# hyx1999/SAM-Decoding

Measured on AMD Instinct MI355X. Metric: tokens/sec (+ mean accepted tokens), Vicuna-7B bs=1, samd_sam_only draft+verify, higher is better.
Workload: dtype f16

## Files before the change

include/samd_hip.h:

```cpp
#ifndef SAMD_HIP_H
#define SAMD_HIP_H

#include <stdint.h>

#ifdef __cplusplus
extern "C" {
#endif

#define SAMD_OK 0
#define SAMD_E_INVALID (-1)
#define SAMD_E_CAPACITY (-2)
#define SAMD_E_HIP (-3)
#define SAMD_E_IO (-4)
#define SAMD_E_NODEVICE (-5)

#define SAMD_MAX_DRAFT 128
#define SAMD_TOPK 8

#define SAMD_REP_DMETA 0
#define SAMD_REP_VERDICT 16
#define SAMD_REP_TOKENS 24
#define SAMD_REP_KVINDEX 152
#define SAMD_REP_COUNTERS 280
#define SAMD_REP_META 288
// ... 135 lines not shown

int samd_session_accept(samd_session_t *s, const int32_t *d_node_argmax, void *stream);
int samd_session_candidates(samd_session_t *s, int64_t *d_candidates, int32_t *d_rowmap, int32_t capacity, void *stream);
int samd_session_step_given(samd_session_t *s, const samd_static_t *sam, const samd_params_t *p, const int32_t *d_best_accept,
                            const int32_t *d_next_token, void *stream);
int samd_session_read_verdict(samd_session_t *s, samd_verdict_host_t *out, void *stream);
int samd_session_commit(samd_session_t *s, const samd_static_t *sam, void *stream);
int samd_session_step(samd_session_t *s, const samd_static_t *sam, const samd_params_t *p,
                      const int32_t *d_node_argmax, void *stream);

int samd_posterior_sampled(const void *d_probs, int32_t dtype, const int64_t *d_candidates, int32_t n_candidates, int32_t depth, int64_t vocab,
                           const double *d_uniforms, int32_t n_uniforms, void *d_work, int32_t *d_out, void *stream);
int samd_posterior_sampled_nodes(const void *d_probs, int32_t dtype, const int32_t *d_rowmap, int32_t n_rows, const int64_t *d_candidates,
                                 int32_t n_candidates, int32_t depth, int64_t vocab, const double *d_uniforms, int32_t n_uniforms,
                                 void *d_work, int32_t *d_out, void *stream);
int samd_kv_compact(samd_session_t *s, void *const *d_tensors, int32_t n_tensors, int32_t n_heads, int64_t max_len,
                    int32_t head_dim, int32_t elem_bytes, void *stream);

int samd_kv_compact_indices(void *const *d_tensors, int32_t n_tensors, int32_t n_heads, int64_t max_len, int32_t head_dim,
                            int32_t elem_bytes, int32_t start, const int32_t *d_indices, int32_t accept, void *stream);

int samd_session_set_cache_length(samd_session_t *s, int32_t length, void *stream);
int samd_session_get_cache_length(samd_session_t *s, int32_t *h_out, void *stream);

typedef struct samd_warm {
    const void *d_packed_w;
    int32_t N, K, splits;
    int32_t kb_per_workgroup;
    int32_t delay;
    int32_t where;
} samd_warm_t;

int64_t samd_tree_attention_workspace(int32_t n_q_pad, int32_t n_heads, int32_t head_dim);
int samd_tree_attention(const void *d_q, const void *d_k_cache, const void *d_v_cache, void *d_out, int32_t dtype,
                        int32_t n_q_pad, int32_t n_heads, int32_t n_kv_heads, int32_t head_dim, int64_t max_len,
                        const uint64_t *d_mask, const int32_t *d_cache_length, const int32_t *d_n, float scale,
                        void *d_workspace, int64_t workspace_bytes, void *stream);
int samd_tree_attention_vt(const void *d_q, const void *d_k_cache, const void *d_vt_cache, void *d_out, int32_t dtype,
                           int32_t n_q_pad, int32_t n_heads, int32_t n_kv_heads, int32_t head_dim, int64_t max_len,
                           const uint64_t *d_mask, const int32_t *d_cache_length, const int32_t *d_n, float scale,
                           void *d_workspace, int64_t workspace_bytes, const samd_warm_t *next, void *stream);
int samd_tree_attention_warm(const void *d_q, const void *d_k_cache, const void *d_v_cache, void *d_out, int32_t dtype,
                             int32_t n_q_pad, int32_t n_heads, int32_t n_kv_heads, int32_t head_dim, int64_t max_len,
                             const uint64_t *d_mask, const int32_t *d_cache_length, const int32_t *d_n, float scale,
                             void *d_workspace, int64_t workspace_bytes, const samd_warm_t *next, void *stream);

// ... 177 lines not shown
```

sam-decoding_amd/csrc/sam_device.h:

```cpp
#pragma once
#include <hip/hip_runtime.h>
#include "samd_common.h"

#define WAVE 64
#define PATH_PAD 255

__device__ __forceinline__ int lane_id() { return threadIdx.x & (WAVE - 1); }

__device__ __forceinline__ void wave_mem_sync() { __builtin_amdgcn_fence(__ATOMIC_SEQ_CST, "workgroup"); }

__device__ __forceinline__ int spill_search(const SamEdge *tab, int deg, int tok) {
    const uint32_t m = samd_spill_slots(deg);
    uint32_t h = samd_spill_hash(tok, m);
    for (uint32_t probes = 0; probes < m; probes++) {
        const SamEdge e = tab[h];
        if (e.tok == tok) return e.dst;
        if (e.tok == -1) return -1;
        h = (h + 1) & (m - 1);
    }
    return -1;
}

__device__ __forceinline__ int st_transfer(const StaticDev &S, int &idx, int &len, int tok) {
    int visited = 0;
// ... 752 lines not shown
            type = 0;
            if (md >= ms || !have_static) {
                int a = id;
                if (a != 0) {
                    const int maxlen = D.meta[M_MAXLEN];
                    int to_end = maxlen - D.minend[a];
                    while (D.link[a] != 0 && P.n_predicts > to_end) { a = D.link[a]; to_end = maxlen - D.minend[a]; }
                }
                n = seq_draft_fixed(sh, D.text, D.meta[M_NTEXT], D.minend[a], P.n_predicts, start);
            } else {
                n = seq_draft_fixed(sh, S.text, S.n_text, S.nodes[is].aux, P.n_predicts, start);
            }
        } else {
            type = 2; n = 1;
            if (lane_id() == 0) { sh.tokens[0] = start; sh.parent[0] = -1; }
            __syncthreads();
        }
    }
    int nl, mxd;
    build_buffers(sh, n, 0, nl, mxd);
    store_draft(D, sh, type, n, nl, mxd, id, md, is, ms, 0);
}

__device__ __forceinline__ void do_accept(const SessionDev &D, StepShared &sh, const int *node_argmax, int type, int n,
                                          int n_leaves, int max_depth, int &accept_out, int &next_token_out) {
    const int i = lane_id();
    for (int k = i; k < n; k += WAVE) sh.node_argmax[k] = node_argmax[k];
    __syncthreads();
    int key = -1;
    for (int row = i; row < n_leaves; row += WAVE) {
        int acc = 0;
        for (int j = 1; j < max_depth; j++) {
            const int cj = sh.path[row][j], pj = sh.path[row][j - 1];
            const int cand = cj == PATH_PAD ? 0 : sh.tokens[cj];
            const int am = sh.node_argmax[pj == PATH_PAD ? n - 1 : pj];
            if (cand != am) break;
            acc++;
        }
        const int kk = acc * SAMD_MAX_DRAFT + (SAMD_MAX_DRAFT - 1 - row);
        key = kk > key ? kk : key;
    }
    for (int o = 32; o > 0; o >>= 1) { int v = __shfl_xor(key, o); key = v > key ? v : key; }
    const int best_acc = key / SAMD_MAX_DRAFT, best = SAMD_MAX_DRAFT - 1 - (key % SAMD_MAX_DRAFT);
    const int a = best_acc + 1;
    for (int k = i; k < a; k += WAVE) {
        const int node = sh.path[best][k];
        const int tk = node == PATH_PAD ? 0 : sh.tokens[node];
        sh.accepted[k] = tk;
        D.acc_tokens[k] = tk;
        D.kv_index[k] = node == PATH_PAD ? -1 : node;
    }
    const int nn_raw = sh.path[best][best_acc];
    const int nn = nn_raw == PATH_PAD ? n - 1 : nn_raw;
    const int next_token = sh.node_argmax[nn];
    if (i == 0) {
        const int start = D.cache_length[0];
        D.verdict[V_BEST] = best; D.verdict[V_ACCEPT] = a; D.verdict[V_NEXT_NODE] = nn; D.verdict[V_NEXT_TOKEN] = next_token;
        D.verdict[V_KV_START] = start; D.verdict[V_IS_TREE] = (type != 0);
        D.cache_length[0] = start + a;
        D.start_token[0] = next_token;
        D.counters[C_STEPS] += 1; D.counters[C_TOKENS] += a;
        D.counters[type == 0 ? C_SEQ_STEPS : C_TREE_STEPS] += 1;
    }
    __syncthreads();
    accept_out = a; next_token_out = next_token;
}

__device__ __forceinline__ void do_accept_given(const SessionDev &D, StepShared &sh, const int *given, const int *next_token_ptr, int type, int n,
                                                int n_leaves, int max_depth, int &accept_out, int &next_token_out) {
    const int i = lane_id();
    int best = given[0], a = given[1];
    best = best < 0 ? 0 : (best >= n_leaves ? (n_leaves > 0 ? n_leaves - 1 : 0) : best);
    a = a < 1 ? 1 : (a > max_depth ? max_depth : a);
    for (int k = i; k < a; k += WAVE) {
        const int node = sh.path[best][k];
        const int tk = node == PATH_PAD ? 0 : sh.tokens[node];
        sh.accepted[k] = tk;
        D.acc_tokens[k] = tk;
        D.kv_index[k] = node == PATH_PAD ? -1 : node;
    }
    const int nn_raw = sh.path[best][a - 1];
    const int nn = nn_raw == PATH_PAD ? n - 1 : nn_raw;
    const int next_token = next_token_ptr[0];
    if (i == 0) {
        const int start = D.cache_length[0];
        D.verdict[V_BEST] = best; D.verdict[V_ACCEPT] = a; D.verdict[V_NEXT_NODE] = nn; D.verdict[V_NEXT_TOKEN] = next_token;
        D.verdict[V_KV_START] = start; D.verdict[V_IS_TREE] = (type != 0);
        D.cache_length[0] = start + a;
        D.start_token[0] = next_token;
        D.counters[C_STEPS] += 1; D.counters[C_TOKENS] += a;
        D.counters[type == 0 ? C_SEQ_STEPS : C_TREE_STEPS] += 1;
    }
    __syncthreads();
    accept_out = a; next_token_out = next_token;
}
```

sam-decoding_amd/csrc/sam_kernels.hip:

```cpp
#include <hip/hip_runtime.h>
#include <cstdio>
#include <cstdlib>
#include <cstring>
#include <ctime>
#include <functional>
#include <vector>
#include <hipcub/hipcub.hpp>
#include "sam_device.h"

#define HIPCHK(x) do { hipError_t e_ = (x); if (e_ != hipSuccess) { samd_set_error("%s: %s", #x, hipGetErrorString(e_)); return SAMD_E_HIP; } } while (0)
#define LAUNCHCHK() do { hipError_t e_ = hipGetLastError(); if (e_ != hipSuccess) { samd_set_error("kernel launch: %s", hipGetErrorString(e_)); return SAMD_E_HIP; } } while (0)

static inline StaticDev static_view(const samd_static_t *s) {
    StaticDev v;
    if (!s) { memset(&v, 0, sizeof(v)); return v; }
    v.nodes = s->d_nodes; v.root_next = s->d_root; v.spill = s->d_spill; v.text = s->d_text;
    v.n_states = (int32_t)s->n_states; v.vocab = (int32_t)s->vocab; v.n_text = (int32_t)s->n_text; v.kind = s->kind;
    v.chain = (const uint4 *)s->d_chain; v.chain_w = samd_chain_w(s->vocab);
    v.root16 = (const uint4 *)s->d_root16; v.bigram = (const uint4 *)s->d_d1hash; v.bigram_mask = s->n_d1hash > 0 ? (uint32_t)(s->n_d1hash - 1) : 0u;
    v.rc_bits = (const uint32_t *)s->d_rc_bits;
    v.ehash = (const uint4 *)s->d_ehash; v.edge_mask = s->n_ehash > 0 ? (uint32_t)(s->n_ehash - 1) : 0u;
    v.topk_cnt = (const int32_t *)s->d_topk_cnt;
    v.hot = s->d_d1hash ? (const uint4 *)s->d_hot : nullptr; v.blocks = s->d_d1hash ? (const uint4 *)s->d_blocks : nullptr; v.eb_tok_bits = samd_eb_tok_bits(s->vocab);
    return v;
// ... 75 lines not shown
    const int32_t *node_argmax;
    const int32_t *given;
    const int32_t *given_next;
    int index, match, start, source, type, reverse;
    int c0, c1, c2, c3;
    int have_static;
    int only_if_deferred;
    int push_report;
};

__device__ __forceinline__ void load_draft(const SessionDev &D, StepShared &sh, int &type, int &n, int &nl, int &md) {
    const int i = lane_id();
    type = D.dmeta[D_TYPE]; n = D.dmeta[D_N]; nl = D.dmeta[D_NLEAVES]; md = D.dmeta[D_MAXDEPTH];
    for (int k = i; k < n; k += WAVE) { sh.tokens[k] = D.tokens[k]; sh.parent[k] = D.parent[k]; }
    path_fill(sh, nl < SAMD_MAX_DRAFT ? (nl < 1 ? 1 : nl) : SAMD_MAX_DRAFT);
    __syncthreads();
    for (int k = i; k < nl * md; k += WAVE) {
        const int v = D.retrieve[k];
        sh.path[k / md][k % md] = v < 0 ? PATH_PAD : (unsigned char)v;
    }
    __syncthreads();
}

__global__ __launch_bounds__(64) void k_session(SessionDev D, StaticDev S, samd_params_t P, StepArgs A) {
    __shared__ StepShared sh;
    const int lane = lane_id();

    if (A.ops & OP_RESET) {
        for (uint32_t k = lane; k <= D.hmask; k += WAVE) D.hkey[k] = SAMD_HEMPTY;
        if (lane == 0) {
            D.link[0] = -1; D.length[0] = 0; D.minend[0] = 0; D.head[0] = -1; D.tail[0] = -1;
            D.text[0] = -1;
            for (int k = 0; k < M_COUNT; k++) D.meta[k] = 0;
            D.meta[M_NSTATES] = 1; D.meta[M_NTEXT] = 1;
            for (int k = 0; k < D_COUNT; k++) D.dmeta[k] = 0;
            for (int k = 0; k < V_COUNT; k++) D.verdict[k] = 0;
            for (int k = 0; k < C_COUNT; k++) D.counters[k] = 0;
            D.start_token[0] = 0; D.cache_length[0] = 0;
        }
        wave_mem_sync();
    }
    if (A.ops & OP_SET_CURSORS) {
        if (lane == 0) { D.meta[M_CUR_IDX] = A.c0; D.meta[M_CUR_LEN] = A.c1; D.meta[M_ST_IDX] = A.c2; D.meta[M_ST_LEN] = A.c3; }
        wave_mem_sync();
    }
    int n_in = A.d_n ? A.d_n[0] : A.n;
    unsigned long long t_prev = __builtin_amdgcn_s_memrealtime();
    auto phase_done = [&](int slot) {
// ... 65 lines not shown
    if (A.ops & OP_DRAFT_FIXED) {
        int n;
        if (A.source == 0) {
            int a = A.index;
            if (a != 0) {
                const int maxlen = D.meta[M_MAXLEN];
                int to_end = maxlen - D.minend[a];
                while (D.link[a] != 0 && P.n_predicts > to_end) { a = D.link[a]; to_end = maxlen - D.minend[a]; }
            }
            n = seq_draft_fixed(sh, D.text, D.meta[M_NTEXT], D.minend[a], P.n_predicts, A.start);
            if (lane == 0) D.dmeta[9] = a;
        } else {
            n = seq_draft_fixed(sh, S.text, S.n_text, S.nodes[A.index].aux, P.n_predicts, A.start);
        }
        int nl, mxd; build_buffers(sh, n, 0, nl, mxd);
        store_draft(D, sh, 0, n, nl, mxd, A.index, 0, A.index, 0, 0);
    }
    if ((A.ops & OP_SET_DRAFT) && !(A.only_if_deferred && D.dmeta[D_TYPE] != 2)) {
        for (int k = lane; k < A.n; k += WAVE) { sh.tokens[k] = A.tokens[k]; sh.parent[k] = A.parents[k]; }
        __syncthreads();
        int nl, mxd; build_buffers(sh, A.n, A.reverse, nl, mxd);
        store_draft(D, sh, A.type, A.n, nl, mxd, 0, 0, 0, 0, A.reverse);
    }
    if (A.push_report && D.h_report) {
        wave_mem_sync();
        for (int k = lane; k < SAMD_REPORT_INTS; k += WAVE)
            __hip_atomic_store(D.h_report + k, D.dmeta[k], __ATOMIC_RELAXED, __HIP_MEMORY_SCOPE_SYSTEM);
        __builtin_amdgcn_fence(__ATOMIC_RELEASE, "");
        asm volatile("s_waitcnt vmcnt(0)" ::: "memory");
        if (lane == 0) {
            const int seq = D.push_seq[0] + 1;
            D.push_seq[0] = seq;
            __hip_atomic_store(D.h_report + SAMD_REPORT_INTS, seq, __ATOMIC_RELEASE, __HIP_MEMORY_SCOPE_SYSTEM);
        }
    }
}

__global__ __launch_bounds__(64) void k_tree_buffers(const int32_t *parent, int n, int reverse, int32_t *position, uint64_t *mask,
                                                     uint8_t *mask_bool, int32_t *retrieve, int32_t *shape) {
    __shared__ StepShared sh;
    const int i = lane_id();
    for (int k = i; k < n; k += WAVE) sh.parent[k] = parent[k];
    __syncthreads();
    int nl, md; build_buffers(sh, n, reverse, nl, md);
    for (int k = i; k < n; k += WAVE) {
        if (position) position[k] = sh.position[k];
        if (mask) { mask[k] = sh.mask[k]; if (n > 64) mask[n + k] = sh.mask_hi[k]; }
        if (mask_bool) for (int j = 0; j < n; j++) mask_bool[(size_t)k * n + j] = (uint8_t)(((j < 64 ? sh.mask[k] >> j : sh.mask_hi[k] >> (j - 64))) & 1ull);
    }
    if (retrieve) for (int k = i; k < nl * md; k += WAVE) { const unsigned char v = sh.path[k / md][k % md]; retrieve[k] = v == PATH_PAD ? -1 : (int)v; }
    if (shape && i == 0) { shape[0] = nl; shape[1] = md; }
}

__global__ __launch_bounds__(64) void k_scripted_argmax(SessionDev D, const int32_t *__restrict__ target, int n_target, int vocab,
                                                        int32_t *__restrict__ out) {
    __shared__ int tok[SAMD_MAX_DRAFT], par[SAMD_MAX_DRAFT];
    const int i = lane_id();
    const int n = D.dmeta[D_N];
// ... 561 lines not shown
    if (!d_visited) return SAMD_E_INVALID;
    return walk_streams(sam, d_cursors, d_tokens, B, T, commit, nullptr, d_visited, stream);
}

int samd_session_create(int32_t max_tokens, samd_session_t **out) {
    if (!out || max_tokens < 1 || max_tokens > (1 << 24)) { samd_set_error("samd_session_create: invalid max_tokens"); return SAMD_E_INVALID; }
    if (samd_device_count() < 1) { samd_set_error("no HIP device"); return SAMD_E_NODEVICE; }
    samd_session_t *s = (samd_session_t *)calloc(1, sizeof(samd_session_t));
    if (!s) { samd_set_error("out of host memory"); return SAMD_E_CAPACITY; }
    s->max_tokens = max_tokens;
    SessionDev &D = s->dev;
    D.max_tokens = max_tokens;
    D.cap_states = 2 * max_tokens + 2;
    D.cap_text = max_tokens + 2;
    uint32_t H = 1024; while (H < (uint32_t)max_tokens * 8u) H <<= 1;
    D.hmask = H - 1;
    size_t off = 0;
    auto carve = [&](size_t bytes) { size_t o = off; off = align_up(off + bytes, 256); return o; };
    const size_t o_link = carve(4ull * D.cap_states), o_len = carve(4ull * D.cap_states), o_me = carve(4ull * D.cap_states),
                 o_head = carve(4ull * D.cap_states), o_tail = carve(4ull * D.cap_states), o_hk = carve(8ull * H),
                 o_hd = carve(4ull * H), o_hn = carve(4ull * H), o_text = carve(4ull * D.cap_text),
                 o_tok = carve(4 * SAMD_MAX_DRAFT), o_par = carve(4 * SAMD_MAX_DRAFT), o_pos = carve(4 * SAMD_MAX_DRAFT), o_mask = carve(8 * 2 * SAMD_MAX_DRAFT),
                 o_ret = carve(4 * SAMD_MAX_DRAFT * SAMD_MAX_DRAFT),
                 o_rep = carve(4 * SAMD_REPORT_INTS), o_st = carve(4), o_cl = carve(4), o_seq = carve(4);
    s->arena_bytes = off;
    if (hipMalloc(&s->arena, off) != hipSuccess) { free(s); samd_set_error("hipMalloc(session arena) failed"); return SAMD_E_HIP; }
    char *base = (char *)s->arena;
    D.link = (int32_t *)(base + o_link); D.length = (int32_t *)(base + o_len); D.minend = (int32_t *)(base + o_me);
    D.head = (int32_t *)(base + o_head); D.tail = (int32_t *)(base + o_tail); D.hkey = (uint64_t *)(base + o_hk);
    D.hdst = (int32_t *)(base + o_hd); D.hnext = (int32_t *)(base + o_hn); D.text = (int32_t *)(base + o_text);
    D.tokens = (int32_t *)(base + o_tok); D.parent = (int32_t *)(base + o_par);
    D.position = (int32_t *)(base + o_pos); D.mask = (uint64_t *)(base + o_mask); D.mask_hi = D.mask + SAMD_MAX_DRAFT; D.retrieve = (int32_t *)(base + o_ret);
    int32_t *rep = (int32_t *)(base + o_rep);
    D.dmeta = rep + SAMD_REP_DMETA; D.verdict = rep + SAMD_REP_VERDICT; D.acc_tokens = rep + SAMD_REP_TOKENS;
    D.kv_index = rep + SAMD_REP_KVINDEX; D.counters = rep + SAMD_REP_COUNTERS; D.meta = rep + SAMD_REP_META;
    D.start_token = (int32_t *)(base + o_st); D.cache_length = (int32_t *)(base + o_cl);
    D.push_seq = (int32_t *)(base + o_seq); D.h_report = nullptr;
    if (hipMemset(s->arena, 0, off) != hipSuccess) { (void)hipFree(s->arena); free(s); return SAMD_E_HIP; }
    *out = s;
    int32_t *target = nullptr;
    int rc = samd_session_report_target(s, &target);
    if (rc == SAMD_OK) rc = samd_session_reset(s, nullptr);
    if (rc == SAMD_OK && hipStreamSynchronize(nullptr) != hipSuccess) rc = SAMD_E_HIP;
    if (rc) { samd_session_free(s); *out = nullptr; }
    return rc;
}

void samd_session_free(samd_session_t *s) {
    if (!s) return;
    if (s->arena) (void)hipFree(s->arena);
    if (s->h_report_host) (void)hipHostFree(s->h_report_host);
    free(s);
}

int samd_session_report_target(samd_session_t *s, int32_t **out_host) {
    if (!s || !out_host) return SAMD_E_INVALID;
    if (!s->h_report_host) {
        void *h = nullptr, *d = nullptr;
        const size_t bytes = 4 * (SAMD_REPORT_INTS + 16);
        if (hipHostMalloc(&h, bytes, hipHostMallocCoherent | hipHostMallocMapped) != hipSuccess) { samd_set_error("hipHostMalloc(report target) failed"); return SAMD_E_HIP; }
// ... 9 lines not shown
int samd_report_wait(const int32_t *h_report, int32_t last_seq, int64_t timeout_us) {
    if (!h_report) return SAMD_E_INVALID;
    const volatile int32_t *seq = h_report + SAMD_REPORT_INTS;
    timespec t0; clock_gettime(CLOCK_MONOTONIC, &t0);
    for (unsigned spin = 0;; spin++) {
        if (*seq != last_seq) { __atomic_thread_fence(__ATOMIC_ACQUIRE); return SAMD_OK; }
        __builtin_ia32_pause();
        if ((spin & 1023u) == 1023u) {
            timespec t; clock_gettime(CLOCK_MONOTONIC, &t);
            if ((t.tv_sec - t0.tv_sec) * 1000000ll + (t.tv_nsec - t0.tv_nsec) / 1000 > timeout_us) return SAMD_E_CAPACITY;
        }
    }
}

static int launch_session(samd_session_t *s, const samd_static_t *sam, const samd_params_t *p, StepArgs &A, void *stream) {
    if (!s) { samd_set_error("null session"); return SAMD_E_INVALID; }
    if (sam && !sam->uploaded) { samd_set_error("static automaton not uploaded"); return SAMD_E_INVALID; }
    samd_params_t P; memset(&P, 0, sizeof(P));
    if (p) P = *p;
    if (p && (P.max_predicts > SAMD_MAX_DRAFT || P.n_predicts > SAMD_MAX_DRAFT || P.max_predicts < 0 || P.n_predicts < 0)) {
        samd_set_error("max_predicts / n_predicts must be in [0, %d]", SAMD_MAX_DRAFT); return SAMD_E_INVALID;
    }
    A.have_static = sam ? 1 : 0;
    hipLaunchKernelGGL(k_session, dim3(1), dim3(WAVE), 0, (hipStream_t)stream, s->dev, static_view(sam), P, A);
    LAUNCHCHK();
    return SAMD_OK;
}

int samd_session_reset(samd_session_t *s, void *stream) {
    StepArgs A; memset(&A, 0, sizeof(A)); A.ops = OP_RESET;
    return launch_session(s, nullptr, nullptr, A, stream);
}

int samd_dyn_add_tokens(samd_session_t *s, const int32_t *d_tokens, int32_t n, const int32_t *d_n, void *stream) {
    if (n < 0 || (!d_tokens && n > 0)) return SAMD_E_INVALID;
    StepArgs A; memset(&A, 0, sizeof(A)); A.ops = OP_ADD; A.tokens = d_tokens; A.n = n; A.d_n = d_n;
    return launch_session(s, nullptr, nullptr, A, stream);
}

int samd_dyn_walk(samd_session_t *s, const int32_t *d_tokens, int32_t n, int32_t commit, int32_t *d_out, void *stream) {
    if (n < 0 || (!d_tokens && n > 0)) return SAMD_E_INVALID;
    StepArgs A; memset(&A, 0, sizeof(A)); A.ops = OP_DYN_WALK; A.tokens = d_tokens; A.n = n; A.commit = commit; A.out2 = d_out;
    return launch_session(s, nullptr, nullptr, A, stream);
}

int samd_session_static_walk(samd_session_t *s, const samd_static_t *sam, const int32_t *d_tokens, int32_t n,
                             const int32_t *d_n, int32_t commit, int32_t *d_out, void *stream) {
// ... 147 lines not shown
        D2H(hk.data(), D.hkey, 8 * H); D2H(hd.data(), D.hdst, 4 * H); D2H(hn.data(), D.hnext, 4 * H); D2H(head.data(), D.head, 4ull * ns);
        HIPCHK(hipStreamSynchronize((hipStream_t)stream));
        size_t k = 0;
        for (int st = 0; st < ns; st++) {
            int d = 0;
            for (int e = head[st]; e >= 0; e = hn[e]) {
                if (h_edge_tok) h_edge_tok[k] = (int32_t)(uint32_t)hk[e];
                if (h_edge_dst) h_edge_dst[k] = hd[e];
                k++; d++;
            }
            if (h_deg) h_deg[st] = d;
        }
    }
    HIPCHK(hipStreamSynchronize((hipStream_t)stream));
    return SAMD_OK;
}

int samd_session_set_cache_length(samd_session_t *s, int32_t length, void *stream) {
    if (!s || length < 0) return SAMD_E_INVALID;
    HIPCHK(hipMemsetD32Async((hipDeviceptr_t)s->dev.cache_length, length, 1, (hipStream_t)stream));
    return SAMD_OK;
}

int samd_session_get_cache_length(samd_session_t *s, int32_t *h_out, void *stream) {
    if (!s || !h_out) return SAMD_E_INVALID;
    D2H(h_out, s->dev.cache_length, 4);
    HIPCHK(hipStreamSynchronize((hipStream_t)stream));
    return SAMD_OK;
}

int samd_scripted_argmax(samd_session_t *s, const int32_t *d_target, int32_t n_target, int32_t vocab, int32_t *d_out, void *stream) {
    if (!s || !d_target || !d_out || n_target < 0 || vocab < 4) return SAMD_E_INVALID;
    hipLaunchKernelGGL(k_scripted_argmax, dim3(1), dim3(WAVE), 0, (hipStream_t)stream, s->dev, d_target, n_target, vocab, d_out);
    LAUNCHCHK();
    return SAMD_OK;
}

static int scripted_logits(samd_session_t *s, const int32_t *d_argmax, void *d_logits, int32_t dtype, int32_t rows, int64_t row_stride, int32_t markov_vocab,
                           int order, void *stream) {
    if (!s || !d_argmax || !d_logits || markov_vocab < 4 || row_stride < markov_vocab) return SAMD_E_INVALID;
    hipStream_t st = (hipStream_t)stream;
#define SCRIPTED(T) do { if (order == 2) hipLaunchKernelGGL((k_scripted_logits<T, 2>), dim3(SAMD_MAX_DRAFT), dim3(WAVE), 0, st, s->dev, d_argmax, (T *)d_logits, (long long)row_stride, markov_vocab, rows); \
                         else hipLaunchKernelGGL((k_scripted_logits<T, 1>), dim3(SAMD_MAX_DRAFT), dim3(WAVE), 0, st, s->dev, d_argmax, (T *)d_logits, (long long)row_stride, markov_vocab, rows); } while (0)
    if (dtype == SAMD_F16) SCRIPTED(_Float16);
    else if (dtype == SAMD_BF16) SCRIPTED(__bf16);
    else if (dtype == SAMD_F32) SCRIPTED(float);
// ... 26 lines not shown
```

sam-decoding_amd/csrc/samd_common.h:

```cpp
#pragma once
#include <stdint.h>
#include <stddef.h>
#include "../../include/samd_hip.h"

#define SAMD_ABI_VERSION 2
#define SAMD_INLINE_EDGES 5
#define SAMD_SPILL_HEAD 3

#define SAMD_SINGLE 0x40000000
#define SAMD_RUN 0x20000000
#define SAMD_LEN_MASK 0x1FFFFFFF
struct __attribute__((aligned(64))) SamNode {
    int32_t link, length, e0_tok, e0_dst;
    int32_t aux, deg, e1_tok, e1_dst;
    int32_t e2_tok, e2_dst, e3_tok, e3_dst;
    int32_t e4_tok, e4_dst, spill, reserved;
};
static_assert(sizeof(SamNode) == 64, "SamNode must be one 64-byte line");
#define SAMD_EDGE_WORD(k) ((k) == 0 ? 2 : 4 + 2 * (k))

struct SamEdge { int32_t tok, dst; };

#if defined(__HIPCC__)
#define SAMD_HD __host__ __device__
// ... 60 lines not shown
enum { C_STEPS = 0, C_TOKENS, C_SEQ_STEPS, C_TREE_STEPS, C_T_ACCEPT, C_T_DYN, C_T_STATIC, C_T_DRAFT, C_COUNT = 8 };

#define SAMD_HEMPTY 0xFFFFFFFFFFFFFFFFull

struct SessionDev {
    int32_t *link, *length, *minend, *head, *tail;
    uint64_t *hkey;
    int32_t *hdst, *hnext;
    int32_t *text;
    int32_t *meta;
    int32_t *tokens, *parent, *position;
    uint64_t *mask;
    uint64_t *mask_hi;
    int32_t *retrieve;
    int32_t *dmeta;
    int32_t *verdict;
    int32_t *acc_tokens, *kv_index;
    int32_t *start_token, *cache_length;
    int32_t *counters;
    uint32_t hmask;
    int32_t cap_states, cap_text, max_tokens;
    int32_t *h_report;
    int32_t *push_seq;
};

struct samd_session {
    SessionDev dev;
    void *arena;
    size_t arena_bytes;
    int32_t max_tokens;
    int32_t *h_report_host;
};

struct samd_static {
    int32_t kind;
    int64_t n_states, n_edges, n_spill, vocab, n_text;
    SamNode *h_nodes;
    int32_t *h_root;
    SamEdge *h_spill;
    int32_t *h_text;
    SamNode *d_nodes;
    int32_t *d_root;
    SamEdge *d_spill;
    int32_t *d_text;
    int uploaded;
    int borrowed;
    void *d_chain;
// ... 58 lines not shown
```

sam-decoding_amd/samd_hip/__init__.py:

```python
import ctypes as C
import os

import numpy as np

_HERE = os.path.dirname(os.path.abspath(__file__))
LIB_PATH = os.environ.get("SAMD_HIP_LIB") or os.path.join(_HERE, "libsamd_hip.so")
MAX_DRAFT = 128
TILE_ROWS = 64
TOPK = 8
REP_DMETA, REP_VERDICT, REP_TOKENS, REP_KVINDEX, REP_COUNTERS, REP_META, REPORT_INTS = 0, 16, 24, 152, 280, 288, 304
KIND_COUNT, KIND_ENDPOS = 0, 1
F16, BF16, F32 = 0, 1, 2

_lib = None


class SamdError(RuntimeError):
    pass


class Params(C.Structure):
    _fields_ = [("variant", C.c_int32), ("max_predicts", C.c_int32), ("alpha", C.c_double), ("K", C.c_int32),
                ("len_bias", C.c_int32), ("n_predicts", C.c_int32), ("len_threshold", C.c_int32),
                ("static_null", C.c_int32), ("reserved", C.c_int32)]
# ... 76 lines not shown
    "samd_embed_rows_ssq": (C.c_int, [_VP, _VP, _VP, _VP, _I32, _I32, _I32, _I32, _VP]),
    "samd_embed_rows_ssq_rope": (C.c_int, [_VP, _VP, _VP, _VP, _I32, _I32, _I32, _I32, _VP, _VP, _VP, _VP, _VP, _I32, _I32, _I32, _VP]),
    "samd_gemm_qkv_rope_norm": (C.c_int, [_VP, _VP, _VP, C.c_float, _VP, _I32, _I32, _VP, _VP, _VP, _VP, _VP, _VP, _I32, _I32, _I32, _I64, _I32, _VP]),
    "samd_gemm_qkv_rope_norm_vt": (C.c_int, [_VP, _VP, _VP, C.c_float, _VP, _I32, _I32, _VP, _VP, _VP, _VP, _VP, _VP, _I32, _I32, _I32, _I64, _I32, _VP]),
    "samd_gemm_pairs_silu_norm": (C.c_int, [_VP, _VP, _VP, C.c_float, _VP, _I32, _I32, _I32, _VP, _I32, _VP]),
    "samd_gemm_cs_residual": (C.c_int, [_VP, _VP, _I32, _I32, _I32, _VP, _VP, _I32, _VP]),
    "samd_gemm_cs_residual_early": (C.c_int, [_VP, _VP, _I32, _I32, _VP, _VP, _I32, _VP, _VP, _I32, _VP]),
    "samd_tree_attention_signal": (C.c_int, [_VP, _VP, _VP, _VP, _I32, _I32, _I32, _I32, _I32, _I64, _VP, _VP, _VP, _F32, _VP, _I64, _VP, _VP]),
    "samd_session_report_target": (C.c_int, [_VP, C.POINTER(_VP)]),
    "samd_report_wait": (C.c_int, [_VP, _I32, _I64]),
    "samd_scripted_logits": (C.c_int, [_VP, _VP, _VP, _I32, _I32, _I64, _I32, _VP]),
    "samd_scripted_logits_order1": (C.c_int, [_VP, _VP, _VP, _I32, _I32, _I64, _I32, _VP]),
    "samd_session_device_views": (C.c_int, [_VP, _VP]),
    "samd_tree_buffers": (C.c_int, [_VP, _I32, _I32, _VP, _VP, _VP, _VP, _VP, _VP]),
    "samd_argmax_rows": (C.c_int, [_VP, _I32, _I32, _I64, _I64, _VP, _VP, _VP]),
    "samd_session_accept": (C.c_int, [_VP, _VP, _VP]),
    "samd_session_read_verdict": (C.c_int, [_VP, _VP, _VP]),
    "samd_session_commit": (C.c_int, [_VP, _VP, _VP]),
    "samd_session_step": (C.c_int, [_VP, _VP, _VP, _VP, _VP]),
    "samd_session_step_given": (C.c_int, [_VP, _VP, _VP, _VP, _VP, _VP]),
    "samd_session_candidates": (C.c_int, [_VP, _VP, _VP, _I32, _VP]),
    "samd_session_set_cache_length": (C.c_int, [_VP, _I32, _VP]),
    "samd_session_get_cache_length": (C.c_int, [_VP, _VP, _VP]),
    "samd_kv_compact": (C.c_int, [_VP, _VP, _I32, _I32, _I64, _I32, _I32, _VP]),
    "samd_kv_compact_indices": (C.c_int, [_VP, _I32, _I32, _I64, _I32, _I32, _I32, _VP, _I32, _VP]),
    "samd_tree_attention_workspace": (_I64, [_I32, _I32, _I32]),
    "samd_tree_attention": (C.c_int, [_VP, _VP, _VP, _VP, _I32, _I32, _I32, _I32, _I32, _I64, _VP, _VP, _VP, _F32,
                                      _VP, _I64, _VP]),
    "samd_tree_attention_vt": (C.c_int, [_VP, _VP, _VP, _VP, _I32, _I32, _I32, _I32, _I32, _I64, _VP, _VP, _VP, _F32,
                                         _VP, _I64, _VP, _VP]),
    "samd_tree_attention_warm": (C.c_int, [_VP, _VP, _VP, _VP, _I32, _I32, _I32, _I32, _I32, _I64, _VP, _VP, _VP, _F32,
                                           _VP, _I64, _VP, _VP]),
    "samd_rope_rows": (C.c_int, [_VP, _VP, _VP, _VP, _VP, _I32, _I32, _I32, _VP]),
    "samd_attention_block": (C.c_int, [_VP, _I32, _I64, _VP, _VP, _VP, _VP, _I32, _I32, _I32, _I32, _I32, _I64, _VP, _VP, _VP, _VP, _F32, _VP]),
    "samd_tree_attention_rope_workspace": (_I64, [_I32, _I32, _I32]),
    "samd_tree_attention_rope": (C.c_int, [_VP, _I32, _I64, _VP, _VP, _VP, _VP, _I32, _I32, _I32, _I32, _I32, _I64, _VP, _VP, _VP, _F32, _VP, _I64, _VP]),
    "samd_rope_kv_write_cs": (C.c_int, [_VP, _VP, _VP, _VP, _VP, _VP, _VP, _VP, _I32, _I32, _I32, _I32, _I64, _I32, _I32, _I64, _VP]),
    "samd_rope_kv_write_cs_vt": (C.c_int, [_VP, _VP, _VP, _VP, _VP, _VP, _VP, _VP, _I32, _I32, _I32, _I32, _I64, _I32, _I32, _I64, _VP]),
    "samd_rope_kv_write_vt": (C.c_int, [_VP, _VP, _VP, _VP, _VP, _VP, _VP, _VP, _VP, _I32, _I32, _I32, _I32, _I64, _I32, _I32, _I32, _I64, _VP]),
    "samd_rope_kv_write_epi": (C.c_int, [_VP, _VP, _VP, _VP, _VP, _VP, _VP, _VP, _VP, _VP, _I32, _I32, _I32, _I32, _I32, _I64, _I32, _I32, _I32, _I64,
                                         _VP, _VP]),
    "samd_kv_compact_vt": (C.c_int, [_VP, _VP, _I32, _I32, _I32, _I64, _I32, _I32, _VP]),
    "samd_kv_compact_indices_vt": (C.c_int, [_VP, _I32, _I32, _I32, _I64, _I32, _I32, _I32, _VP, _I32, _VP]),
    "samd_posterior_sampled": (C.c_int, [_VP, _I32, _VP, _I32, _I32, _I64, _VP, _I32, _VP, _VP, _VP]),
    "samd_posterior_sampled_nodes": (C.c_int, [_VP, _I32, _VP, _I32, _VP, _I32, _I32, _I64, _VP, _I32, _VP, _VP, _VP]),
    "samd_e2_rowstats_workspace": (C.c_int64, [_I64]),
# ... 361 lines not shown

    def read_verdict(self):
        out = VerdictHost()
        check(lib().samd_session_read_verdict(self._h, C.byref(out), current_stream()))
        return out

    def commit(self, sam):
        check(lib().samd_session_commit(self._h, sam._h if sam is not None else None, current_stream()))

    def step(self, sam, params, d_node_argmax):
        check(lib().samd_session_step(self._h, sam._h if sam is not None else None, C.byref(params), _ptr(d_node_argmax),
                                      current_stream()))

    def candidates(self, d_candidates, d_rowmap):
        check(lib().samd_session_candidates(self._h, _ptr(d_candidates), _ptr(d_rowmap), d_rowmap.numel(), current_stream()))

    def step_given(self, sam, params, d_best_accept, d_next_token):
        check(lib().samd_session_step_given(self._h, sam._h if sam is not None else None, C.byref(params), _ptr(d_best_accept), _ptr(d_next_token),
                                            current_stream()))

    def set_cache_length(self, length):
        check(lib().samd_session_set_cache_length(self._h, int(length), current_stream()))

    def get_cache_length(self):
        out = C.c_int32()
        check(lib().samd_session_get_cache_length(self._h, C.byref(out), current_stream()))
        return out.value

    def kv_compact(self, d_tensor_ptrs, n_tensors, n_heads, max_len, head_dim, elem_bytes, n_transposed=0):
        check(lib().samd_kv_compact_vt(self._h, _ptr(d_tensor_ptrs), n_tensors, n_transposed, n_heads, max_len, head_dim, elem_bytes, current_stream()))

    def device_views(self):
        if self._views is None:
            out = (C.c_void_p * 16)()
            check(lib().samd_session_device_views(self._h, out))
            names = ("tokens", "parent", "position", "mask", "retrieve", "dmeta", "verdict", "acc_tokens", "kv_index",
                     "start_token", "cache_length", "history", "counters", "meta")
            self._views = {k: out[i] for i, k in enumerate(names)}
        return self._views

    def export(self, with_edges=True):
        info = (C.c_int64 * 10)()
        check(lib().samd_session_export(self._h, info, None, None, None, None, None, None, None, current_stream()))
        ns, ne, nt = info[0], info[1], info[2]
        link, length, minend, deg = (np.empty(ns, np.int32) for _ in range(4))
        et, ed, text = np.empty(ne, np.int32), np.empty(ne, np.int32), np.empty(nt, np.int32)
# ... 42 lines not shown
```

Before: 814.0.

## Split fused session step across two workgroups for dynamic and static SAM drafting

Launches the fused accept/commit/draft session kernel with two single-wave workgroups. One updates the dynamic automaton and does the dynamic lookup while the other walks the static automaton and builds the static tree draft, and the two meet through an atomic arrival counter. The static side publishes its tree into a global scratch area so the last workgroup to arrive picks the better draft and stores it. The aim is to take the static-SAM work off the serial critical path of the per-step single-wave kernel, at the cost of a cross-workgroup handoff, extra global traffic and added timing counters.

Measured after the change: 817.0 (median of 6 runs). About the same (+0.4%).

```diff
diff --git a/include/samd_hip.h b/include/samd_hip.h
--- a/include/samd_hip.h
+++ b/include/samd_hip.h
@@ -181,6 +181,7 @@
 
 int samd_session_set_cache_length(samd_session_t *s, int32_t length, void *stream);
 int samd_session_get_cache_length(samd_session_t *s, int32_t *h_out, void *stream);
+int samd_session_split_stats(samd_session_t *s, int32_t *h_out, void *stream);
 
 typedef struct samd_warm {
     const void *d_packed_w;
diff --git a/sam-decoding_amd/csrc/sam_device.h b/sam-decoding_amd/csrc/sam_device.h
--- a/sam-decoding_amd/csrc/sam_device.h
+++ b/sam-decoding_amd/csrc/sam_device.h
@@ -798,6 +798,7 @@
     store_draft(D, sh, type, n, nl, mxd, id, md, is, ms, 0);
 }
 
+template <bool STORE = true>
 __device__ __forceinline__ void do_accept(const SessionDev &D, StepShared &sh, const int *node_argmax, int type, int n,
                                           int n_leaves, int max_depth, int &accept_out, int &next_token_out) {
     const int i = lane_id();
@@ -823,13 +824,12 @@
         const int node = sh.path[best][k];
         const int tk = node == PATH_PAD ? 0 : sh.tokens[node];
         sh.accepted[k] = tk;
-        D.acc_tokens[k] = tk;
-        D.kv_index[k] = node == PATH_PAD ? -1 : node;
+        if (STORE) { D.acc_tokens[k] = tk; D.kv_index[k] = node == PATH_PAD ? -1 : node; }
     }
     const int nn_raw = sh.path[best][best_acc];
     const int nn = nn_raw == PATH_PAD ? n - 1 : nn_raw;
     const int next_token = sh.node_argmax[nn];
-    if (i == 0) {
+    if (STORE && i == 0) {
         const int start = D.cache_length[0];
         D.verdict[V_BEST] = best; D.verdict[V_ACCEPT] = a; D.verdict[V_NEXT_NODE] = nn; D.verdict[V_NEXT_TOKEN] = next_token;
         D.verdict[V_KV_START] = start; D.verdict[V_IS_TREE] = (type != 0);
@@ -842,6 +842,7 @@
     accept_out = a; next_token_out = next_token;
 }
 
+template <bool STORE = true>
 __device__ __forceinline__ void do_accept_given(const SessionDev &D, StepShared &sh, const int *given, const int *next_token_ptr, int type, int n,
                                                 int n_leaves, int max_depth, int &accept_out, int &next_token_out) {
     const int i = lane_id();
@@ -852,13 +853,12 @@
         const int node = sh.path[best][k];
         const int tk = node == PATH_PAD ? 0 : sh.tokens[node];
         sh.accepted[k] = tk;
-        D.acc_tokens[k] = tk;
-        D.kv_index[k] = node == PATH_PAD ? -1 : node;
+        if (STORE) { D.acc_tokens[k] = tk; D.kv_index[k] = node == PATH_PAD ? -1 : node; }
     }
     const int nn_raw = sh.path[best][a - 1];
     const int nn = nn_raw == PATH_PAD ? n - 1 : nn_raw;
     const int next_token = next_token_ptr[0];
-    if (i == 0) {
+    if (STORE && i == 0) {
         const int start = D.cache_length[0];
         D.verdict[V_BEST] = best; D.verdict[V_ACCEPT] = a; D.verdict[V_NEXT_NODE] = nn; D.verdict[V_NEXT_TOKEN] = next_token;
         D.verdict[V_KV_START] = start; D.verdict[V_IS_TREE] = (type != 0);
diff --git a/sam-decoding_amd/csrc/sam_kernels.hip b/sam-decoding_amd/csrc/sam_kernels.hip
--- a/sam-decoding_amd/csrc/sam_kernels.hip
+++ b/sam-decoding_amd/csrc/sam_kernels.hip
@@ -121,8 +121,146 @@
     __syncthreads();
 }
 
+__device__ __forceinline__ void push_report(const SessionDev &D) {
+    const int lane = lane_id();
+    wave_mem_sync();
+    for (int k = lane; k < SAMD_REPORT_INTS; k += WAVE)
+        __hip_atomic_store(D.h_report + k, D.dmeta[k], __ATOMIC_RELAXED, __HIP_MEMORY_SCOPE_SYSTEM);
+    __builtin_amdgcn_fence(__ATOMIC_RELEASE, "");
+    asm volatile("s_waitcnt vmcnt(0)" ::: "memory");
+    if (lane == 0) {
+        const int seq = D.push_seq[0] + 1;
+        D.push_seq[0] = seq;
+        __hip_atomic_store(D.h_report + SAMD_REPORT_INTS, seq, __ATOMIC_RELEASE, __HIP_MEMORY_SCOPE_SYSTEM);
+    }
+}
+
+__device__ __forceinline__ void session_split_step(const SessionDev &D, const StaticDev &S, const samd_params_t &P, const StepArgs &A, StepShared &sh) {
+    const int lane = lane_id();
+    const bool dyn_side = blockIdx.x == 0;
+    int32_t *sp = D.split;
+    const unsigned long long t_entry = __builtin_amdgcn_s_memrealtime();
+    unsigned long long t_prev = t_entry;
+    auto lap = [&]() { const unsigned long long t = __builtin_amdgcn_s_memrealtime(); const int d = (int)(t - t_prev); t_prev = t; return d; };
+    int type, n, nl, mxd, a, start;
+    load_draft(D, sh, type, n, nl, mxd);
+    int id = 0, md = 0, t_lookup = 0;
+    int is = 0, ms = 0, st_idx = 0, st_len = 0, t_static = 0, t_draft = 0;
+    int tn = 0, tnl = 0, tmd = 0;
+    bool early = false;
+    if (dyn_side) {
+        if (A.ops & OP_ACCEPT) do_accept(D, sh, A.node_argmax, type, n, nl, mxd, a, start);
+        else do_accept_given(D, sh, A.given, A.given_next, type, n, nl, mxd, a, start);
+        wave_mem_sync();
+        const int t_accept = lap();
+        dyn_add_tokens(D, sh.accepted, a);
+        wave_mem_sync();
+        const int t_dyn = lap();
+        id = D.meta[M_CUR_IDX]; md = D.meta[M_CUR_LEN];
+        dyn_transfer(D, id, md, start);
+        t_lookup = lap();
+        if (lane == 0) {
+            D.counters[C_T_ACCEPT] += t_accept; D.counters[C_T_DYN] += t_dyn;
+            sp[SPLIT_ID] = id; sp[SPLIT_MD] = md; sp[SPLIT_T_DRAFT_DYN] = t_lookup; sp[SPLIT_T_SIDE_DYN] = (int)(t_prev - t_entry);
+        }
+    } else {
+        if (A.ops & OP_ACCEPT) do_accept<false>(D, sh, A.node_argmax, type, n, nl, mxd, a, start);
+        else do_accept_given<false>(D, sh, A.given, A.given_next, type, n, nl, mxd, a, start);
+        is = D.meta[M_ST_IDX]; ms = D.meta[M_ST_LEN];
+        (void)lap();
+        st_transfer_tokens(S, is, ms, sh.accepted, a);
+        st_idx = is; st_len = ms;
+        t_static = lap();
+        st_transfer(S, is, ms, start);
+        ms -= P.len_bias;
+        if (ms > 0) {
+            tn = tree_draft(sh, S, is, draft_size(ms, P.alpha, P.max_predicts), P.K, start);
+            build_buffers(sh, tn, 0, tnl, tmd);
+        }
+        int seen = 0;
+        if (lane == 0) seen = __hip_atomic_load(D.split_arrive, __ATOMIC_RELAXED, __HIP_MEMORY_SCOPE_AGENT);
+        early = (__shfl(seen, 0) & 1) != 0;
+        if (!early) {
+            if (tn > 0) {
+                unsigned long long *m64 = reinterpret_cast<unsigned long long *>(sp + SPLIT_MASK);
+                for (int k = lane; k < tn; k += WAVE) {
+                    sp[SPLIT_TOKENS + k] = sh.tokens[k]; sp[SPLIT_PARENT + k] = sh.parent[k]; sp[SPLIT_POSITION + k] = sh.position[k];
+                    m64[k] = sh.mask[k]; m64[SAMD_MAX_DRAFT + k] = sh.mask_hi[k];
+                }
+                const int upr = (tmd + 15) >> 4;
+                uint4 *pp = reinterpret_cast<uint4 *>(sp + SPLIT_PATH);
+                for (int k = lane; k < tnl * upr; k += WAVE) {
+                    const int r = k / upr, u = k % upr;
+                    pp[r * (SAMD_MAX_DRAFT / 16) + u] = reinterpret_cast<const uint4 *>(&sh.path[r][0])[u];
+                }
+            }
+            t_draft = lap();
+            if (lane == 0) {
+                sp[SPLIT_N] = tn; sp[SPLIT_NLEAVES] = tnl; sp[SPLIT_MAXDEPTH] = tmd; sp[SPLIT_IS] = is; sp[SPLIT_MS] = ms;
+                sp[SPLIT_ST_IDX] = st_idx; sp[SPLIT_ST_LEN] = st_len; sp[SPLIT_T_STATIC] = t_static; sp[SPLIT_T_DRAFT_ST] = t_draft;
+            }
+        } else t_draft = lap();
+    }
+    const int t_side = (int)(t_prev - t_entry);
+    int old = 1;
+    if (early) {
+        if (lane == 0) (void)__hip_atomic_fetch_add(D.split_arrive, 1, __ATOMIC_RELAXED, __HIP_MEMORY_SCOPE_AGENT);
+    } else {
+        __builtin_amdgcn_fence(__ATOMIC_RELEASE, "agent");
+        asm volatile("s_waitcnt vmcnt(0)" ::: "memory");
+        if (lane == 0) old = __hip_atomic_fetch_add(D.split_arrive, 1, __ATOMIC_RELAXED, __HIP_MEMORY_SCOPE_AGENT);
+        old = __shfl(old, 0);
+        if (!(old & 1)) return;
+    }
+    __builtin_amdgcn_fence(__ATOMIC_ACQUIRE, "agent");
+    int t_side_other;
+    if (dyn_side) {
+        is = sp[SPLIT_IS]; ms = sp[SPLIT_MS]; st_idx = sp[SPLIT_ST_IDX]; st_len = sp[SPLIT_ST_LEN]; t_static = sp[SPLIT_T_STATIC]; t_draft = sp[SPLIT_T_DRAFT_ST];
+        tn = sp[SPLIT_N]; tnl = sp[SPLIT_NLEAVES]; tmd = sp[SPLIT_MAXDEPTH];
+        t_side_other = t_static + t_draft;
+    } else {
+        id = sp[SPLIT_ID]; md = sp[SPLIT_MD]; t_lookup = sp[SPLIT_T_DRAFT_DYN]; t_side_other = sp[SPLIT_T_SIDE_DYN];
+    }
+    const int t_join = lap();
+    int otype, on, onl, omd;
+    if (md >= ms) {
+        otype = 0;
+        on = seq_draft_var(sh, D.text, D.meta[M_NTEXT], D.minend[id], draft_size(md, P.alpha, P.max_predicts), start);
+        build_buffers(sh, on, 0, onl, omd);
+    } else {
+        otype = 1; on = tn; onl = tnl; omd = tmd;
+        if (dyn_side) {
+            const unsigned long long *m64 = reinterpret_cast<const unsigned long long *>(sp + SPLIT_MASK);
+            for (int k = lane; k < on; k += WAVE) {
+                sh.tokens[k] = sp[SPLIT_TOKENS + k]; sh.parent[k] = sp[SPLIT_PARENT + k]; sh.position[k] = sp[SPLIT_POSITION + k];
+                sh.mask[k] = m64[k]; sh.mask_hi[k] = m64[SAMD_MAX_DRAFT + k];
+            }
+            const int upr = (omd + 15) >> 4;
+            const uint4 *pp = reinterpret_cast<const uint4 *>(sp + SPLIT_PATH);
+            for (int k = lane; k < onl * upr; k += WAVE) {
+                const int r = k / upr, u = k % upr;
+                reinterpret_cast<uint4 *>(&sh.path[r][0])[u] = pp[r * (SAMD_MAX_DRAFT / 16) + u];
+            }
+            __syncthreads();
+        }
+    }
+    store_draft(D, sh, otype, on, onl, omd, id, md, is, ms, 0);
+    const int t_finish = lap();
+    if (lane == 0) {
+        D.meta[M_ST_IDX] = st_idx; D.meta[M_ST_LEN] = st_len;
+        D.counters[C_T_STATIC] += t_static;
+        D.counters[C_T_DRAFT] += t_lookup + t_draft + t_join + t_finish;
+        sp[SPLIT_STAT_STEPS] += 1; sp[SPLIT_STAT_ST_LAST] += dyn_side ? 0 : 1; sp[SPLIT_STAT_ST_EARLY] += early ? 1 : 0;
+        sp[SPLIT_STAT_T_SIDE_DYN] += dyn_side ? t_side : t_side_other; sp[SPLIT_STAT_T_SIDE_ST] += dyn_side ? t_side_other : t_side;
+        sp[SPLIT_STAT_T_JOIN] += t_join; sp[SPLIT_STAT_T_FINISH] += t_finish;
+    }
+    wave_mem_sync();
+    if (A.push_report && D.h_report) push_report(D);
+}
+
 __global__ __launch_bounds__(64) void k_session(SessionDev D, StaticDev S, samd_params_t P, StepArgs A) {
     __shared__ StepShared sh;
+    if (gridDim.x == 2) { session_split_step(D, S, P, A, sh); return; }
     const int lane = lane_id();
 
     if (A.ops & OP_RESET) {
@@ -234,18 +372,7 @@
         int nl, mxd; build_buffers(sh, A.n, A.reverse, nl, mxd);
         store_draft(D, sh, A.type, A.n, nl, mxd, 0, 0, 0, 0, A.reverse);
     }
-    if (A.push_report && D.h_report) {
-        wave_mem_sync();
-        for (int k = lane; k < SAMD_REPORT_INTS; k += WAVE)
-            __hip_atomic_store(D.h_report + k, D.dmeta[k], __ATOMIC_RELAXED, __HIP_MEMORY_SCOPE_SYSTEM);
-        __builtin_amdgcn_fence(__ATOMIC_RELEASE, "");
-        asm volatile("s_waitcnt vmcnt(0)" ::: "memory");
-        if (lane == 0) {
-            const int seq = D.push_seq[0] + 1;
-            D.push_seq[0] = seq;
-            __hip_atomic_store(D.h_report + SAMD_REPORT_INTS, seq, __ATOMIC_RELEASE, __HIP_MEMORY_SCOPE_SYSTEM);
-        }
-    }
+    if (A.push_report && D.h_report) push_report(D);
 }
 
 __global__ __launch_bounds__(64) void k_tree_buffers(const int32_t *parent, int n, int reverse, int32_t *position, uint64_t *mask,
@@ -853,7 +980,8 @@
                  o_hd = carve(4ull * H), o_hn = carve(4ull * H), o_text = carve(4ull * D.cap_text),
                  o_tok = carve(4 * SAMD_MAX_DRAFT), o_par = carve(4 * SAMD_MAX_DRAFT), o_pos = carve(4 * SAMD_MAX_DRAFT), o_mask = carve(8 * 2 * SAMD_MAX_DRAFT),
                  o_ret = carve(4 * SAMD_MAX_DRAFT * SAMD_MAX_DRAFT),
-                 o_rep = carve(4 * SAMD_REPORT_INTS), o_st = carve(4), o_cl = carve(4), o_seq = carve(4);
+                 o_rep = carve(4 * SAMD_REPORT_INTS), o_st = carve(4), o_cl = carve(4), o_seq = carve(4),
+                 o_split = carve(4 * SPLIT_WORDS), o_arrive = carve(4);
     s->arena_bytes = off;
     if (hipMalloc(&s->arena, off) != hipSuccess) { free(s); samd_set_error("hipMalloc(session arena) failed"); return SAMD_E_HIP; }
     char *base = (char *)s->arena;
@@ -867,6 +995,7 @@
     D.kv_index = rep + SAMD_REP_KVINDEX; D.counters = rep + SAMD_REP_COUNTERS; D.meta = rep + SAMD_REP_META;
     D.start_token = (int32_t *)(base + o_st); D.cache_length = (int32_t *)(base + o_cl);
     D.push_seq = (int32_t *)(base + o_seq); D.h_report = nullptr;
+    D.split = (int32_t *)(base + o_split); D.split_arrive = (int32_t *)(base + o_arrive);
     if (hipMemset(s->arena, 0, off) != hipSuccess) { (void)hipFree(s->arena); free(s); return SAMD_E_HIP; }
     *out = s;
     int32_t *target = nullptr;
@@ -922,7 +1051,10 @@
         samd_set_error("max_predicts / n_predicts must be in [0, %d]", SAMD_MAX_DRAFT); return SAMD_E_INVALID;
     }
     A.have_static = sam ? 1 : 0;
-    hipLaunchKernelGGL(k_session, dim3(1), dim3(WAVE), 0, (hipStream_t)stream, s->dev, static_view(sam), P, A);
+    const bool fused = A.ops == (OP_ACCEPT | OP_COMMIT | OP_DRAFT) || A.ops == (OP_ACCEPT_GIVEN | OP_COMMIT | OP_DRAFT);
+    bool split = fused && sam && P.variant == 0;
+    if (split) { const char *e = getenv("SAMD_SESSION_SPLIT"); split = !(e && e[0] == '0' && e[1] == 0); }
+    hipLaunchKernelGGL(k_session, dim3(split ? 2 : 1), dim3(WAVE), 0, (hipStream_t)stream, s->dev, static_view(sam), P, A);
     LAUNCHCHK();
     return SAMD_OK;
 }
@@ -1116,6 +1248,13 @@
     return SAMD_OK;
 }
 
+int samd_session_split_stats(samd_session_t *s, int32_t *h_out, void *stream) {
+    if (!s || !h_out) return SAMD_E_INVALID;
+    D2H(h_out, s->dev.split + SPLIT_STAT, 4 * SPLIT_STAT_COUNT);
+    HIPCHK(hipStreamSynchronize((hipStream_t)stream));
+    return SAMD_OK;
+}
+
 int samd_session_get_cache_length(samd_session_t *s, int32_t *h_out, void *stream) {
     if (!s || !h_out) return SAMD_E_INVALID;
     D2H(h_out, s->dev.cache_length, 4);
diff --git a/sam-decoding_amd/csrc/samd_common.h b/sam-decoding_amd/csrc/samd_common.h
--- a/sam-decoding_amd/csrc/samd_common.h
+++ b/sam-decoding_amd/csrc/samd_common.h
@@ -106,7 +106,16 @@
     int32_t cap_states, cap_text, max_tokens;
     int32_t *h_report;
     int32_t *push_seq;
+    int32_t *split;
+    int32_t *split_arrive;
 };
+enum { SPLIT_N = 0, SPLIT_NLEAVES, SPLIT_MAXDEPTH, SPLIT_IS, SPLIT_MS, SPLIT_ST_IDX, SPLIT_ST_LEN, SPLIT_T_STATIC, SPLIT_T_DRAFT_ST,
+       SPLIT_ID = 32, SPLIT_MD, SPLIT_T_DRAFT_DYN, SPLIT_T_SIDE_DYN,
+       SPLIT_STAT = 48, SPLIT_STAT_STEPS = SPLIT_STAT, SPLIT_STAT_ST_LAST, SPLIT_STAT_ST_EARLY, SPLIT_STAT_T_SIDE_DYN, SPLIT_STAT_T_SIDE_ST,
+       SPLIT_STAT_T_JOIN, SPLIT_STAT_T_FINISH, SPLIT_STAT_COUNT = 8, SPLIT_HDR = 64,
+       SPLIT_TOKENS = SPLIT_HDR, SPLIT_PARENT = SPLIT_TOKENS + SAMD_MAX_DRAFT, SPLIT_POSITION = SPLIT_PARENT + SAMD_MAX_DRAFT,
+       SPLIT_MASK = SPLIT_POSITION + SAMD_MAX_DRAFT, SPLIT_PATH = SPLIT_MASK + 4 * SAMD_MAX_DRAFT,
+       SPLIT_WORDS = SPLIT_PATH + SAMD_MAX_DRAFT * SAMD_MAX_DRAFT / 4 };
 
 struct samd_session {
     SessionDev dev;
diff --git a/sam-decoding_amd/samd_hip/__init__.py b/sam-decoding_amd/samd_hip/__init__.py
--- a/sam-decoding_amd/samd_hip/__init__.py
+++ b/sam-decoding_amd/samd_hip/__init__.py
@@ -122,6 +122,7 @@
     "samd_session_candidates": (C.c_int, [_VP, _VP, _VP, _I32, _VP]),
     "samd_session_set_cache_length": (C.c_int, [_VP, _I32, _VP]),
     "samd_session_get_cache_length": (C.c_int, [_VP, _VP, _VP]),
+    "samd_session_split_stats": (C.c_int, [_VP, _VP, _VP]),
     "samd_kv_compact": (C.c_int, [_VP, _VP, _I32, _I32, _I64, _I32, _I32, _VP]),
     "samd_kv_compact_indices": (C.c_int, [_VP, _I32, _I32, _I64, _I32, _I32, _I32, _VP, _I32, _VP]),
     "samd_tree_attention_workspace": (_I64, [_I32, _I32, _I32]),
@@ -529,6 +530,13 @@
     def set_cache_length(self, length):
         check(lib().samd_session_set_cache_length(self._h, int(length), current_stream()))
 
+    def split_stats(self):
+        out = (C.c_int32 * 8)()
+        check(lib().samd_session_split_stats(self._h, out, current_stream()))
+        steps = max(1, out[0])
+        return dict(steps=out[0], static_side_finished=out[1], static_side_skipped_handover=out[2], dyn_side_us=out[3] / steps / 100.0,
+                    static_side_us=out[4] / steps / 100.0, join_us=out[5] / steps / 100.0, finish_us=out[6] / steps / 100.0)
+
     def get_cache_length(self):
         out = C.c_int32()
         check(lib().samd_session_get_cache_length(self._h, C.byref(out), current_stream()))
```
